# huangnengCSU/longcallR

Measured on AMD Instinct MI355X. Metric: candidate_sites_per_sec, higher is better.
Workload: dtype u8 in, u32 counts, f64 likelihoods, i64 fixed-point phase scores

## Files before the change

### longcallr_amd/csrc/k4_enum.hip

```cpp
#include <climits>
#include <type_traits>
#include "k4_dev.h"
#include "k4_kernels.h"

#ifndef ENUM_OCC
#define ENUM_OCC 3
#endif
namespace {

struct EnumTile { int32_t slot; uint32_t e0, ne; };
__device__ __forceinline__ EnumTile enum_tile_of(const PhaseDev& P, const EnumSpan* __restrict__ spans, int n_spans, uint32_t per, bool winner) {
  EnumTile t;
  const uint32_t bid = blockIdx.x;
  if (winner) { t.slot = spans[bid].slot; t.e0 = 0; t.ne = 1; return t; }
  const int lane = threadIdx.x & 63;
  int lo = 0, hi = n_spans;
  if (n_spans <= 4096) {
    const int step = (n_spans + 63) / 64;
    const int i1 = lane * step;
    const unsigned long long m1 = __ballot(i1 < n_spans && spans[min(i1, n_spans - 1)].tile0 <= bid);
    const int seg = __popcll(m1) - 1;
    lo = seg * step; hi = min(n_spans, lo + step);
    const int i2 = lo + lane;
    const unsigned long long m2 = __ballot(i2 < hi && spans[min(i2, n_spans - 1)].tile0 <= bid);
    lo = lo + __popcll(m2) - 1;
  } else {
    while (hi - lo > 1) { const int mid = (lo + hi) >> 1; if (spans[mid].tile0 <= bid) lo = mid; else hi = mid; }
  }
  t.slot = spans[lo].slot;
  const uint32_t n = 1u << P.reg[t.slot].S;
  t.e0 = (bid - spans[lo].tile0) * per;
  t.ne = min(per, n - t.e0);
  return t;
}

#ifdef ENUM_PROF
#define ENUM_PT(i) do { if (threadIdx.x == 0) atomicMax(&P.tie_ctr[i], (unsigned long long)((long long)wall_clock64() - prof_t0)); } while (0)
#else
#define ENUM_PT(i) do { } while (0)
#endif
__global__ void __launch_bounds__(64 * ENUM_WAVES)
k4_enum_resolve(PhaseDev P, const EnumSpan* __restrict__ spans, const int64_t* __restrict__ job_base, const long long* __restrict__ job_obj,
                const int64_t* __restrict__ st_base, const unsigned long long* __restrict__ st_words) {
  extern __shared__ __attribute__((aligned(16))) uint8_t lds[];
  const long long prof_t0 = (long long)wall_clock64(); (void)prof_t0;
  const int slot = spans[blockIdx.x].slot;
  const RegionDev rd = P.reg[slot];
  const int tid = threadIdx.x, nt = blockDim.x, lane = tid & 63, wave = tid >> 6;
  const int R = rd.R, S = rd.S;
  const uint32_t E = (uint32_t)P.prow_ptr[rd.rp_off + R];
  const uint32_t n_jobs = 1u << S;
// ... 359 lines not shown
  if (tid == 0) s_prof = 0;
  __syncthreads();
  if (tid == 0 && dif) s_prof = ((unsigned long long)(((long long)wall_clock64() - prof_t5) & 0xfffff) << 24) | ((unsigned long long)min(max(max(s_tloc[0], s_tloc[1]), max(s_tloc[2], s_tloc[3])) >> 4, 4095u) << 12) | min(max(max(s_tfull[0], s_tfull[1]), max(s_tfull[2], s_tfull[3])) >> 4, 4095u);
#endif
  const uint32_t we = s_win;
  const unsigned long long m0 = ld_st(we, nk);
  const uint32_t dneg = (uint32_t)m0, eta0 = (uint32_t)(m0 >> 32), etap = (uint32_t)ld_st(we, nk + 1);
  for (int i = tid; i < S; i += nt) {
    P.st_delta[rd.snp_off + i] = (int8_t)(((dneg >> i) & 1u) ? -1 : 1);
    P.st_eta[rd.snp_off + i] = (int8_t)(((eta0 >> i) & 1u) ? 0 : (((etap >> i) & 1u) ? 1 : -1));
  }
  for (int row = tid; row < R; row += nt) P.st_sigma[rd.sig_off + row] = (int8_t)(((ld_st(we, (uint32_t)row >> 6) >> (row & 63)) & 1ull) ? -1 : 1);
  if (tid == 0) P.st_obj[slot] = best;
#ifdef ENUM_PROF
  __syncthreads();
  if (tid == 0) atomicMax(&P.tie_ctr[7], ((unsigned long long)(((long long)wall_clock64() - prof_t0) & 0xfffff) << 44) | s_prof);
#endif
}

__device__ __forceinline__ int enum_incl_scan(int v) {
  v += __builtin_amdgcn_update_dpp(0, v, 0x111, 0xf, 0xf, false);
  v += __builtin_amdgcn_update_dpp(0, v, 0x112, 0xf, 0xf, false);
  v += __builtin_amdgcn_update_dpp(0, v, 0x114, 0xf, 0xf, false);
  v += __builtin_amdgcn_update_dpp(0, v, 0x118, 0xf, 0xf, false);
  v += __builtin_amdgcn_update_dpp(0, v, 0x142, 0xa, 0xf, false);
  v += __builtin_amdgcn_update_dpp(0, v, 0x143, 0xc, 0xf, false);
  return v;
}

__device__ __forceinline__ bool enum_tie_row_flips(const int row, const uint32_t sneg, const uint32_t dneg, const uint32_t eta0, const uint32_t etap,
                                                   const uint16_t* rp, const uint16_t* ent16, const double* lut) {
// ... 305 lines not shown
      job_obj[job_base[t.slot] + e] = total;
    }
    wave_lds_sync();
  };
  for (uint32_t kk = wave; kk < ne; kk += ENUM_WAVES) run_restart(t.e0 + kk);
  n_tie_f64 = (uint32_t)wave_sum_ll((long long)n_tie_f64); n_tie_flip = (uint32_t)wave_sum_ll((long long)n_tie_flip); n_tie_unres = (uint32_t)wave_sum_ll((long long)n_tie_unres);
  if (lane == 0) {
    if (n_tie_f64) TIE_COUNT(P.tie_ctr, TIE_SIGMA_F64, (unsigned long long)n_tie_f64);
    if (n_tie_flip) TIE_COUNT(P.tie_ctr, TIE_SIGMA_FLIPS, (unsigned long long)n_tie_flip);
    if (n_tie_unres) TIE_COUNT(P.tie_ctr, TIE_SIGMA_UNRES, (unsigned long long)n_tie_unres);
    if (n_dtie) TIE_COUNT(P.tie_ctr, TIE_DELTA_UNRES, (unsigned long long)n_dtie);
    if (n_step) TIE_COUNT(P.tie_ctr, TIE_STEP_UNRES, (unsigned long long)n_step);
  }
}

__device__ __forceinline__ uint32_t enum_spread8(uint32_t x) { x = (x | (x << 4)) & 0x0F0Fu; x = (x | (x << 2)) & 0x3333u; x = (x | (x << 1)) & 0x5555u; return x; }
__device__ __forceinline__ int enum_mad24(int a, int b, int c) { int d; asm("v_mad_i32_i24 %0, %1, %2, %3" : "=v"(d) : "v"(a), "v"(b), "v"(c)); return d; }

#ifndef ENUM_BITS_OCC
#define ENUM_BITS_OCC 2
#endif
__global__ void __launch_bounds__(64 * ENUM_WAVES, ENUM_BITS_OCC)
k4_enum_bits(PhaseDev P, const EnumSpan* __restrict__ spans, int32_t n_spans, uint32_t per, const int64_t* __restrict__ job_base,
             long long* __restrict__ job_obj, const int64_t* __restrict__ st_base, unsigned long long* __restrict__ st_words,
             long long* __restrict__ region_best, uint32_t* __restrict__ redo, uint32_t redo_cap) {
  extern __shared__ __attribute__((aligned(16))) uint8_t lds[];
  const EnumTile t = enum_tile_of(P, spans, n_spans, per, false);
  const RegionDev rd = P.reg[t.slot];
  const int R = rd.R, S = rd.S;
  const uint32_t E = (uint32_t)P.prow_ptr[rd.rp_off + R];
  const EnumLayout L = enum_layout(R, E, true, (uint32_t)S);
  const int Sp = (int)enum_bits_sp((uint32_t)S);
  uint2* wl2 = (uint2*)lds;
  double* lut = (double*)(lds + L.lut);
  uint2* csr = (uint2*)(lds + L.csr);
  uint32_t* csc = (uint32_t*)(lds + L.csc);
  uint16_t* rp = (uint16_t*)(lds + L.rp); uint16_t* first_row = (uint16_t*)(lds + L.first_row);
  uint16_t* ent16 = (uint16_t*)(lds + L.ent16);
  const int tid = threadIdx.x, nt = blockDim.x;
  const uint32_t c = enum_chunk(E);
  __shared__ long long s_cF[32], s_cW[32], s_cRef[32], s_cVar[32], s_het[32];
  __shared__ uint8_t s_live[32];
  if (tid < 32) {
    const long long w = tid < 31 ? P.lut.f1e[tid] - P.lut.fe[tid] : 0;
    wl2[tid] = make_uint2((uint32_t)w & 0x7fffffu, (uint32_t)(w >> 23) & 0xffffffu);
  }
  if (tid < 64) lut[tid] = (tid & 31) < 31 ? (tid < 32 ? P.lut64->le[tid] : P.lut64->l1e[tid - 32]) : 0.0;
  const int32_t* g_rp = P.prow_ptr + rd.rp_off;
  for (int r = tid; r <= R; r += nt) rp[r] = (uint16_t)g_rp[r];
  __shared__ int32_t cps[33];
  if (tid <= S && tid < 33) cps[tid] = P.ccol_ptr[rd.cp_off + tid];
  int eta_init = 0;
  if (tid < 32) {
    long long cF = 0, cW = 0, cRef = 0, cVar = 0, het = 0; bool live = false;
    if (tid < S) {
      const long long* sc = P.snp_const + 4ll * (rd.snp_off + tid);
      cF = sc[0]; cW = sc[1]; cRef = sc[2] + P.lut.f_homref; cVar = sc[3] + P.lut.f_homvar;
      const int n = P.ccol_ptr[rd.cp_off + tid + 1] - P.ccol_ptr[rd.cp_off + tid];
      het = P.lut.f_het0 - (long long)n * P.lut.f_log2;
      live = P.snp_fp[rd.snp_off + tid] != 0 && n > 0;
      eta_init = init_genotype(P.snp_vt[rd.snp_off + tid]);
    }
    s_cF[tid] = cF; s_cW[tid] = cW; s_cRef[tid] = cRef; s_cVar[tid] = cVar; s_het[tid] = het; s_live[tid] = live ? 1 : 0;
  }
  __shared__ uint32_t s_e0i, s_epi;
  if (tid < 64) {
    const uint32_t a = (uint32_t)__ballot(tid < S && tid < 32 && eta_init == 0), b = (uint32_t)__ballot(tid < S && tid < 32 && eta_init == 1);
    if (tid == 0) { s_e0i = a; s_epi = b; }
  }
  __syncthreads();
  for (int e = tid; e < (int)E; e += nt) {
    const uint32_t cv = P.cval[rd.e_off + e];
    int col = 0;
    for (int i = 0; i < S; i++) col += (int)((uint32_t)e >= (uint32_t)cps[i + 1]);
    csc[e] = (uint32_t)P.crow[rd.e_off + e] | ((uint32_t)col << 16) | ((cv & 32u) << 16) | ((cv & 31u) << 22) | 0x80000000u;
  }
  uint16_t* const perm = (uint16_t*)(lds + L.pos);
  uint16_t* const gof = perm + ((R + 3) & ~3);
  uint16_t* const kidx = (uint16_t*)(lds + L.state);
  __shared__ int s_cnt[3];
  __shared__ int s_lstart[32];
  __syncthreads();
  if (tid < 64) {
// ... 13 lines not shown
#pragma unroll
        for (int Lk = 2; Lk < 32; Lk++) {
          if (Lk <= S) {
            const unsigned long long bm = __ballot(n == Lk);
            if (n == Lk) kidx[r] = (uint16_t)(tot[Lk] + __popcll(bm & lt));
            tot[Lk] += __popcll(bm);
          }
        }
      }
    }
    int mine = 0;
#pragma unroll
    for (int Lk = 2; Lk < 32; Lk++) if (ln == Lk) mine = tot[Lk];
    int longer = 0;
    for (int Lk = 31; Lk >= 2; Lk--) { const int tl = __shfl(mine, Lk, 64); if (ln == Lk) s_lstart[ln] = longer; longer += tl; }
    if (ln == 0) { s_cnt[0] = longer; s_cnt[2] = nS; }
  }
  __syncthreads();
  const int nM = s_cnt[0], nS = s_cnt[2], nG = (nM + 63) >> 6;
  for (int r = tid; r < R; r += nt) {
    const int n = min(31, (int)rp[r + 1] - (int)rp[r]);
    if (n >= 2) perm[s_lstart[n] + kidx[r]] = (uint16_t)r;
  }
  __syncthreads();
  if (tid < 64) {
    int carry = 0;
    for (int g0 = 0; g0 <= nG; g0 += 64) {
      const int g = g0 + tid;
      const int len = g < nG ? min(31, (int)rp[perm[64 * g] + 1] - (int)rp[perm[64 * g]]) : 0;
      const int inc = wave_incl_scan(len);
      if (g <= nG) gof[g] = (uint16_t)(carry + inc - len);
// ... 9 lines not shown
    if (e0 == e1) continue;
    int at, step;
    if (e1 - e0 >= 2) {
      const int k = s_lstart[min(31, e1 - e0)] + kidx[r];
      at = 64 * (int)gof[k >> 6] + (k & 63); step = 64;
    } else { perm[nM + kidx[r]] = (uint16_t)r; at = eM + kidx[r]; step = 1; }
    for (int e = e0; e < e1; e++) {
      const uint32_t v = P.pval[rd.e_off + e];
      const uint32_t meta = (uint32_t)P.pcol[rd.e_off + e] | (v & 32u) | (e + 1 == e1 ? 64u : 0u) | 128u;
      const uint2 w = wl2[v & 31u];
      csr[at + (e - e0) * step] = make_uint2(w.x | (meta << 24), w.y);
      ent16[e] = (uint16_t)((meta & 63u) | ((v & 31u) << 6) | (e + 1 == e1 ? 0x800u : 0u));
    }
  }
  __syncthreads();
  const int lane = tid & 63, wave = tid >> 6;
  uint8_t* const wst = lds + L.state + wave * L.stride;
  uint8_t* const sg8 = wst;
  unsigned long long* const Macc = (unsigned long long*)(wst + ((R + 15) & ~7u));
  uint2* const mt = (uint2*)(Macc + 8 * Sp);
  uint32_t* const ms = (uint32_t*)(mt + 32);
  uint32_t* const tq = ms + 24;
  uint32_t* const tq_n = tq + ENUM_TQ;
  const int c0 = min((int)E, lane * (int)c), c1 = min((int)E, (lane + 1) * (int)c);
  const int n_del = (int)min(c, E);
  const uint32_t smask = S >= 32 ? 0xffffffffu : ((1u << S) - 1u);
  const uint32_t e0_init = s_e0i, ep_init = s_epi;
  const int nk = (R + 63) / 64;
  unsigned long long* const st_reg = st_words + st_base[t.slot];
  const uint32_t stw = enum_state_words((uint32_t)R);
  uint32_t n_tie_f64 = 0, n_tie_flip = 0, n_tie_unres = 0;
  uint32_t n_dtie = 0, n_step = 0;
  const int n_pass = (S + 7) >> 3;
  for (uint32_t g0 = 8u * wave; g0 < t.ne; g0 += 8u * ENUM_WAVES) {
    const uint32_t e_base = t.e0 + g0;
    const int nst = (int)min(8u, t.ne - g0);
    const uint32_t valid8 = (1u << nst) - 1u;
    if (lane < 8) { ms[lane] = (e_base + (uint32_t)lane) & smask; ms[8 + lane] = e0_init; ms[16 + lane] = ep_init; }
    {
      constexpr uint64_t G = 0x9E3779B97F4A7C15ULL;
      const uint64_t RG = (uint64_t)R * G;
      uint64_t a_row = rd.seed + ((uint64_t)S + (uint64_t)R + (uint64_t)e_base * (uint64_t)R + (uint64_t)lane + 1ull) * G;
// ... 179 lines not shown
              alo[s] += __umul24(b, wq[x].x); ahi[s] += __mul24((int)b, whi);
            }
          }
        }
        if (cur >= 0) flush();
      }
      wave_lds_sync();
      uint32_t any2 = 0, chg8 = 0;
      {
        const int s = lane >> 3;
        const uint32_t od = ms[s], oe0 = ms[8 + s], oep = ms[16 + s];
        uint32_t nd = od, ne0 = oe0, nep = oep;
        for (int p = 0; p < n_pass; p++) {
          const int i = 8 * p + (lane & 7);
          const bool in = i < S;
          const bool live = in && s_live[i & 31] != 0;
          int d_new = (int)((od >> i) & 1u), h_new = ((oe0 >> i) & 1u) ? 0 : (((oep >> i) & 1u) ? 1 : -1);
          bool changed = false, dtie = false;
          if (live && ((act >> s) & 1u)) {
            const long long M = (long long)Macc[s * Sp + i];
            const long long cF = s_cF[i], cW = s_cW[i], cRef = s_cRef[i], cVar = s_cVar[i], het = s_het[i];
            const long long N0 = cF + M + het, N1 = cF + cW - M + het;
            int ch = 0; long long nb = N0;
            if (N1 > nb) { ch = 1; nb = N1; }
            if (cRef > nb) { ch = 2; nb = cRef; }
            if (cVar > nb) { ch = 3; nb = cVar; }
            dtie = (int)(N0 == nb) + (int)(N1 == nb) + (int)(cRef == nb) + (int)(cVar == nb) > 1;
            const long long ncur = h_new == 0 ? N0 : (h_new == 1 ? cRef : cVar);
            changed = nb > ncur;
            if (ch == 1) d_new ^= 1;
            h_new = ch <= 1 ? 0 : (ch == 2 ? 1 : -1);
            objl[p] = ch <= 1 ? nb - het : (ch == 2 ? cRef - P.lut.f_homref : cVar - P.lut.f_homvar);
          }
          if (in) Macc[s * Sp + i] = 0;
          const unsigned long long bd = __ballot(in && d_new), b0 = __ballot(in && h_new == 0), bp = __ballot(in && h_new == 1);
          const unsigned long long bc = __ballot(changed), bt = __ballot(dtie);
// ... 95 lines not shown
        }
        if (lane == 0) { stp[nk] = (unsigned long long)ms[s] | ((unsigned long long)ms[8 + s] << 32); stp[nk + 1] = (unsigned long long)ms[16 + s]; stp[nk + 2] = sig; }
      }
      if (lane == 0) job_obj[job_base[t.slot] + e] = total;
    }
    wave_lds_sync();
  }
  n_tie_f64 = (uint32_t)wave_sum_ll((long long)n_tie_f64); n_tie_flip = (uint32_t)wave_sum_ll((long long)n_tie_flip); n_tie_unres = (uint32_t)wave_sum_ll((long long)n_tie_unres);
  if (lane == 0) {
    if (n_tie_f64) TIE_COUNT(P.tie_ctr, TIE_SIGMA_F64, (unsigned long long)n_tie_f64);
    if (n_tie_flip) TIE_COUNT(P.tie_ctr, TIE_SIGMA_FLIPS, (unsigned long long)n_tie_flip);
    if (n_tie_unres) TIE_COUNT(P.tie_ctr, TIE_SIGMA_UNRES, (unsigned long long)n_tie_unres);
    if (n_dtie) TIE_COUNT(P.tie_ctr, TIE_DELTA_UNRES, (unsigned long long)n_dtie);
    if (n_step) TIE_COUNT(P.tie_ctr, TIE_STEP_UNRES, (unsigned long long)n_step);
  }
}

__device__ __forceinline__ void enum_big_restart(const PhaseDev& P, const RegionDev& rd, int slot, uint32_t e, bool winner, int8_t* base, double* qrow,
                                                 long long* red, const long long* wl, unsigned long long* s_sig, const int64_t* __restrict__ job_base,
                                                 long long* __restrict__ job_obj, const int64_t* __restrict__ st_base, unsigned long long* __restrict__ st_words,
                                                 const MatView& mv, unsigned long long* macc = nullptr) {
  int8_t* sg = base; int8_t* dl = base + rd.R; int8_t* et = dl + rd.S;
  const int8_t* vt = P.snp_vt + rd.snp_off;
  const int lane = threadIdx.x & 63, wave = threadIdx.x >> 6;
  const uint32_t nk = (uint32_t)(rd.R + 63) / 64, sw = enum_state_words((uint32_t)rd.R);
  const bool keep = !winner && st_words && st_base[slot] >= 0;
  for (int i = threadIdx.x; i < rd.S; i += blockDim.x) { dl[i] = ((e >> i) & 1u) ? -1 : 1; et[i] = init_genotype(vt[i]); }
  const uint64_t ctr0 = (uint64_t)rd.S + (uint64_t)rd.R + (uint64_t)e * (uint64_t)rd.R;
  for (int row = threadIdx.x; row < rd.R; row += blockDim.x) sg[row] = u01(rd.seed, ctr0 + row) < 0.5 ? -1 : 1;
  __syncthreads();
// ... 173 lines not shown
        }
        __syncthreads();
        win = s_first;
      }
    }
  }
  if (tid == 0) win_e[slot] = win;
}
}

void launch_k4_enum_reg(unsigned n_blocks, size_t dyn_lds, hipStream_t s, const PhaseDev& P, const EnumSpan* spans, int32_t n_spans,
                        uint32_t per, const int64_t* job_base, long long* job_obj, const int64_t* st_base, unsigned long long* st_words,
                        long long* region_best, uint32_t* redo, uint32_t redo_cap) {
  hipLaunchKernelGGL(k4_enum_reg, dim3(n_blocks), dim3(64 * ENUM_WAVES), dyn_lds, s, P, spans, n_spans, per, job_base, job_obj, st_base, st_words, region_best, redo, redo_cap);
}
void launch_k4_enum_bits(unsigned n_blocks, size_t dyn_lds, hipStream_t s, const PhaseDev& P, const EnumSpan* spans, int32_t n_spans,
                         uint32_t per, const int64_t* job_base, long long* job_obj, const int64_t* st_base, unsigned long long* st_words,
                         long long* region_best, uint32_t* redo, uint32_t redo_cap) {
  hipLaunchKernelGGL(k4_enum_bits, dim3(n_blocks), dim3(64 * ENUM_WAVES), dyn_lds, s, P, spans, n_spans, per, job_base, job_obj, st_base, st_words, region_best, redo, redo_cap);
}
hipError_t k4_set_dyn_lds_once(const void* fn, int bytes, int slot);
void launch_k4_enum_redo(unsigned n_blocks, hipStream_t s, const PhaseDev& P, const uint32_t* redo, uint32_t redo_cap, int8_t* scratch, int32_t scratch_stride,
                         double* qrow, int64_t qrow_stride, const int64_t* job_base, long long* job_obj, const int64_t* st_base, unsigned long long* st_words,
                         uint32_t lds_bytes) {
  lds_bytes = std::min<uint32_t>(lds_bytes, 128 * 1024);
  if (lds_bytes > 32 * 1024 && k4_set_dyn_lds_once(reinterpret_cast<const void*>(&k4_enum_redo), 128 * 1024, 6) != hipSuccess) { (void)hipGetLastError(); lds_bytes = 32 * 1024; }
  hipLaunchKernelGGL(k4_enum_redo, dim3(n_blocks), dim3(LCR_BLOCK), lds_bytes, s, P, redo, redo_cap, scratch, scratch_stride, qrow, qrow_stride, job_base, job_obj, st_base, st_words, lds_bytes);
}
void launch_k4_enum_resolve(unsigned n_regions, size_t dyn_lds, hipStream_t s, const PhaseDev& P, const EnumSpan* spans, const int64_t* job_base,
                            const long long* job_obj, const int64_t* st_base, const unsigned long long* st_words) {
  hipLaunchKernelGGL(k4_enum_resolve, dim3(n_regions), dim3(64 * ENUM_WAVES), dyn_lds, s, P, spans, job_base, job_obj, st_base, st_words);
}
void launch_k4_enum_big(unsigned n_blocks, hipStream_t s, const PhaseDev& P, const EnumSpan* spans, int32_t n_spans, uint32_t per,
                        const int64_t* job_base, long long* job_obj, const uint32_t* win_e, const int64_t* st_base, unsigned long long* st_words,
// ... 8 lines not shown
```

### longcallr_amd/csrc/k4_kernels.h

```cpp
#pragma once
#include "k4_types.h"

struct EnumSpan { int32_t slot; uint32_t tile0; };
constexpr int ENUM_WAVES = 4;
constexpr uint32_t ENUM_LDS_MAX = 63 * 1024;

constexpr uint32_t ENUM_TQ = 126;
constexpr uint32_t ENUM_TCAP = 256;
#ifndef ENUM_BITS_PER_V
#define ENUM_BITS_PER_V 64
#endif
constexpr uint32_t ENUM_BITS_PER = ENUM_BITS_PER_V;
__host__ __device__ inline uint32_t enum_bits_sp(uint32_t S) { return (S + 7) & ~7u; }
__host__ __device__ inline uint32_t enum_bits_stride(uint32_t R, uint32_t S) { return ((R + 15) & ~7u) + 8 * 8 * enum_bits_sp(S) + 8 * 32 + 4 * 24 + 4 * (ENUM_TQ + 2); }
struct EnumLayout { uint32_t lut, csr, csc, rp, first_row, ent16, pos, state, stride, total; };
__host__ __device__ inline EnumLayout enum_layout(uint32_t R, uint32_t E, bool bits = false, uint32_t S = 32) {
  EnumLayout L;
  uint32_t o = 256;
  L.lut = o; o += 512;
  L.csr = o; o += 8 * (E + (bits ? 64 * (S < 31 ? S : 31) : 0));
  L.csc = o; o += 4 * E;
  L.rp = o; o += 2 * (R + 1);
  L.first_row = o; o += 2 * 65 + (bits ? 2 * 64 : 0);
  o = (o + 7) & ~7u;
  L.ent16 = o; o += 2 * ((E + 3) & ~3u);
  L.pos = o; if (bits) o += 2 * ((R + 3) & ~3u) + 2 * ((R + 4) & ~3u);
  o = (o + 15) & ~15u;
  L.state = o;
  L.stride = bits ? enum_bits_stride(R, S) : 8 * ((R + 63) / 64 + 1) + 8 * 32 + 4 * (ENUM_TQ + 2);
  o += ENUM_WAVES * L.stride;
  L.total = o;
  return L;
}
__host__ __device__ inline uint32_t enum_state_words(uint32_t R) { return (R + 63) / 64 + 3; }
__host__ __device__ inline uint32_t resolve_tlcap(uint32_t S) { return S >= 12 ? 4096u : (S < 6 ? 64u : (1u << S)); }
struct ResolveLayout { uint32_t lut, rp, ent16, pse, sg_ref, hetw, repmask, rowsnps, res, total; };
__host__ __device__ inline ResolveLayout resolve_layout(uint32_t R, uint32_t E, uint32_t S) {
  ResolveLayout L;
  const uint32_t nk = (R + 63) / 64;
  uint32_t o = 0;
  L.lut = o; o += 512;
  L.rp = o; o += 2 * (R + 2);
  o = (o + 15) & ~15u;
  L.ent16 = o; o += 2 * ((E + 7) & ~7u);
  o = (o + 15) & ~15u;
  L.pse = o; o += 8 * ((E + 8) & ~7u);
  L.sg_ref = o; o += 8 * (nk + 1);
  L.hetw = o; o += 8 * (nk + 1);
  L.repmask = o; o += 8 * nk * (S ? S : 1);
  L.rowsnps = o; o += 4 * (R + 1);
  o = (o + 7) & ~7u;
  L.res = o; o += ENUM_TCAP * 16 + 96 * 10 + 16 + 2 * resolve_tlcap(S);
  L.total = (o + 15) & ~15u;
  return L;
}
__host__ __device__ inline uint32_t enum_chunk(uint32_t E) { return E ? (E + 63) / 64 : 1; }

void launch_k4_enum_reg(unsigned n_blocks, size_t dyn_lds, hipStream_t s, const PhaseDev& P, const EnumSpan* spans, int32_t n_spans,
                        uint32_t per, const int64_t* job_base, long long* job_obj, const int64_t* st_base, unsigned long long* st_words,
                        long long* region_best, uint32_t* redo , uint32_t redo_cap);
void launch_k4_enum_bits(unsigned n_blocks, size_t dyn_lds, hipStream_t s, const PhaseDev& P, const EnumSpan* spans, int32_t n_spans,
                         uint32_t per, const int64_t* job_base, long long* job_obj, const int64_t* st_base, unsigned long long* st_words,
                         long long* region_best, uint32_t* redo, uint32_t redo_cap);
void launch_k4_enum_redo(unsigned n_blocks, hipStream_t s, const PhaseDev& P, const uint32_t* redo, uint32_t redo_cap, int8_t* scratch ,
                         int32_t scratch_stride, double* qrow , int64_t qrow_stride, const int64_t* job_base, long long* job_obj,
                         const int64_t* st_base, unsigned long long* st_words, uint32_t lds_bytes );
void launch_k4_enum_resolve(unsigned n_regions, size_t dyn_lds, hipStream_t s, const PhaseDev& P, const EnumSpan* spans, const int64_t* job_base,
                            const long long* job_obj, const int64_t* st_base, const unsigned long long* st_words);
void launch_k4_enum_big(unsigned n_blocks, hipStream_t s, const PhaseDev& P, const EnumSpan* spans, int32_t n_spans, uint32_t per,
                        const int64_t* job_base, long long* job_obj, const uint32_t* win_e ,
                        const int64_t* st_base , unsigned long long* st_words,
                        double* qrow , int64_t qrow_stride);
void launch_k4_enum_resolve_big(int32_t n, hipStream_t s, const PhaseDev& P, const EnumSpan* spans, const int64_t* job_base, const long long* job_obj,
                                const int64_t* st_base, const unsigned long long* st_words, uint32_t* win_e, double* terms ,
                                int64_t terms_stride);

constexpr int STAGE_THREADS = 256;
constexpr int STG_E = 8192, STG_R = 4096, STG_S = 512;
// ... 26 lines not shown
```

### longcallr_amd/csrc/k4_phase.hip

```cpp
#include <algorithm>
#include <chrono>
#include <cstdio>
#include <cstdlib>
#include <cmath>
#include <cstring>
#include <climits>
#include <map>
#include <thread>
#include <mutex>
#include <fcntl.h>
#include <sys/file.h>
#include <unistd.h>
#include <sys/stat.h>
#include <cerrno>

#include "k4_dev.h"
#include "k4_grid.h"
#include "k4_post.h"
#include "k4_kernels.h"

namespace {


struct HostLut {
// ... 565 lines not shown
    for (size_t k = 0; k < enum_slots.size(); k++) enum_slots[k] = (int32_t)(uint32_t)key[k];
  }
  HT("en:sorted");
  int32_t max_state = 0;
  for (int g : enum_slots) max_state = std::max(max_state, stat[g].R + 2 * in.snps(g));
  const int32_t stride = (max_state + 63) & ~63;
  P.scratch_stride = stride;
  const bool force_big = dbg.enum_force_big != 0;
  const bool force_stream = dbg.enum_force_stream != 0;
  enum { CL_STREAM, CL_BITS, CL_BIG, NCLS };
  std::vector<EnumSpan> spans[NCLS];
  spans[CL_STREAM].reserve(enum_slots.size()); spans[CL_BITS].reserve(enum_slots.size());
  size_t n_t[NCLS] = {0, 0, 0};
  const uint32_t per_of[NCLS] = {ENUM_STREAM_PER_WAVE * ENUM_WAVES, ENUM_BITS_PER, 1u};
  std::vector<int64_t>& job_base = enum_job_base; std::vector<int64_t>& st_base = enum_st_base;
  job_base.assign(ng, 0); st_base.assign(ng, 0);
  int64_t nj = 0, st_words = 0, big_words = 0, big_emax = 0;
  uint32_t lds_need[NCLS] = {0, 0, 0}, res_lds[NCLS] = {0, 0, 0};
  std::vector<int32_t> post_slots, post_slots_b, post_slots_c;
  post_slots.reserve(enum_slots.size());
  for (int g : enum_slots) {
    const int S = in.snps(g);
    const StageStat& st = stat[g];
    const EnumLayout EL_stream = enum_layout(st.R, st.E), EL_bits = enum_layout(st.R, st.E, true, (uint32_t)std::min(S, 32));
    const bool use_bits = !force_stream && S <= 31 && EL_bits.total <= ENUM_LDS_MAX;
    const EnumLayout EL = use_bits ? EL_bits : EL_stream;
    const uint32_t RL = resolve_layout((uint32_t)st.R, (uint32_t)st.E, (uint32_t)S).total;
    int cls = CL_BIG;
    if (!force_big && st.R < 65536 && st.E < 65536 && S <= 31 && EL.total <= ENUM_LDS_MAX && RL <= ENUM_LDS_MAX && st.max_rows <= 64)
      cls = use_bits ? CL_BITS : CL_STREAM;
    if (cls != CL_BIG && (int64_t)((uint64_t)1 << std::min(S, 62)) * enum_state_words((uint32_t)st.R) > ((int64_t)1 << 27)) cls = CL_BIG;
    if (cls != CL_BIG) { lds_need[cls] = std::max(lds_need[cls], EL.total); res_lds[cls] = std::max(res_lds[cls], RL); }
    job_base[g] = nj;
    const uint64_t n = 1ull << S;
    st_base[g] = -1;
    if (cls != CL_BIG) { st_base[g] = st_words; st_words += (int64_t)n * enum_state_words((uint32_t)st.R); }
    else if ((int64_t)n * enum_state_words((uint32_t)st.R) <= ((int64_t)1 << 26) - big_words) {
      st_base[g] = st_words; st_words += (int64_t)n * enum_state_words((uint32_t)st.R); big_words += (int64_t)n * enum_state_words((uint32_t)st.R);
      big_emax = std::max<int64_t>(big_emax, st.E);
    }
    if (n_t[cls] + (n + per_of[cls] - 1) / per_of[cls] > 0x7fffffffull) { if (c.err) *c.err = "too many enumeration restarts for one launch"; return LCR_E_ARG; }
    spans[cls].push_back({g, (uint32_t)n_t[cls]});
    n_t[cls] += (size_t)((n + per_of[cls] - 1) / per_of[cls]);
    nj += (int64_t)n;
    if (!c.host_post[g] && !c.grid_post[g]) (cls == CL_BITS ? post_slots_b : (cls == CL_BIG ? post_slots_c : post_slots)).push_back(g);
    if (c.prof && cls == CL_BIG) fprintf(stderr, "[phase]   global-memory enumeration region %d: R %d E %d S %d max_rows %d max_n %d, LDS image %u B\n", g, st.R, st.E, S, st.max_rows, st.max_n, EL.total);
  }
  if (c.prof) fprintf(stderr, "[phase]   enumeration classes: bit states %zu regions / %zu tiles, streaming %zu / %zu, global %zu / %zu\n",
                      spans[CL_BITS].size(), n_t[CL_BITS], spans[CL_STREAM].size(), n_t[CL_STREAM], spans[CL_BIG].size(), n_t[CL_BIG]);
  size_t n_w[NCLS], s_off[NCLS], n_spans = 0;
  for (int k = 0; k < NCLS; k++) { n_w[k] = spans[k].size(); s_off[k] = n_spans; n_spans += n_w[k]; }
  const size_t ns = enum_slots.size(), nps_a = post_slots.size(), nps_b = post_slots_b.size(), nps_c = post_slots_c.size(), nps = nps_a + nps_b + nps_c;
  const size_t off_jb_al = (n_spans * sizeof(EnumSpan) + 7) & ~(size_t)7;
  const size_t off_sb = off_jb_al + (size_t)ng * 8;
  const size_t up_bytes = off_sb + (size_t)ng * 8 + (ns + nps) * 4;
  HT("en:classes");
  PCHK(d_en_st.reserve((size_t)std::max<int64_t>(st_words, 1) * 8));
  PCHK(d_en_job.reserve(up_bytes + 64));
  PCHK(d_en_obj.reserve((size_t)nj * 8 + (size_t)ng * 8 + (size_t)ng * 8 + 64));
  PCHK(h_en_up.reserve(up_bytes + 64));
  uint8_t* const up = h_en_up.as<uint8_t>();
  for (int k = 0; k < NCLS; k++) memcpy(up + s_off[k] * sizeof(EnumSpan), spans[k].data(), n_w[k] * sizeof(EnumSpan));
  memcpy(up + off_jb_al, job_base.data(), (size_t)ng * 8);
  memcpy(up + off_sb, st_base.data(), (size_t)ng * 8);
  memcpy(up + off_sb + (size_t)ng * 8, enum_slots.data(), ns * 4);
  memcpy(up + off_sb + (size_t)ng * 8 + ns * 4, post_slots.data(), nps_a * 4);
  memcpy(up + off_sb + (size_t)ng * 8 + (ns + nps_a) * 4, post_slots_b.data(), nps_b * 4);
  memcpy(up + off_sb + (size_t)ng * 8 + (ns + nps_a + nps_b) * 4, post_slots_c.data(), nps_c * 4);
  PCHK(hipMemcpyAsync(d_en_job.p, up, up_bytes, hipMemcpyHostToDevice, stream));
  HT("en:up_q");
  const EnumSpan* d_sp = d_en_job.as<EnumSpan>();
  const int64_t* d_jb = (const int64_t*)(d_en_job.as<uint8_t>() + off_jb_al);
  const int64_t* d_sb = (const int64_t*)(d_en_job.as<uint8_t>() + off_sb);
  const int32_t* d_sl = (const int32_t*)(d_en_job.as<uint8_t>() + off_sb + (size_t)ng * 8);
  const int32_t* d_psl = d_sl + ns;
  long long* d_obj = d_en_obj.as<long long>();
  uint32_t* d_win = (uint32_t*)(d_obj + nj);
  const size_t n_big_blocks = std::max(n_t[CL_BIG], n_w[CL_BIG]);
  const bool full_ties = dbg.tie_arith >= 3;
  int32_t max_rows_any = 1;
  for (int g : enum_slots) max_rows_any = std::max(max_rows_any, stat[g].R);
  const int64_t qstride = ((int64_t)2 * max_rows_any + 15) & ~(int64_t)15;
  const size_t n_scr_blocks = n_big_blocks + 2 * (size_t)REDO_GRID;
  PCHK(d_en_scr.reserve((size_t)stride * n_scr_blocks + 64));
  P.scratch = d_en_scr.as<int8_t>();
  if (full_ties) PCHK(d_en_qrow.reserve((size_t)qstride * n_scr_blocks * 8 + 64));
  uint32_t* const redo_a = full_ties ? d_en_redo.as<uint32_t>() : nullptr;
  uint32_t* const redo_b = full_ties ? d_en_redo.as<uint32_t>() + 4 + 2 * REDO_CAP : nullptr;
  double* const qrow_all = full_ties ? d_en_qrow.as<double>() : nullptr;
// ... 7 lines not shown
  long long* const d_rbest = d_en_rbest.as<long long>();
  unsigned long long* const d_st = d_en_st.as<unsigned long long>();
  const uint32_t post_lds = c.post_lds; const PostIn& pin = c.pin; const PostLut& plut = c.plut;
  auto launch = [&](const size_t* cnt, const uint32_t* win) -> hipError_t {
    const bool fork = cnt[CL_STREAM] && (cnt[CL_BITS] || cnt[CL_BIG]);
    hipStream_t const qb = fork ? aux : stream;
    hipError_t e = hipSuccess;
    if (fork) { if ((e = hipEventRecord(ev_fork, stream)) != hipSuccess) return e; if ((e = hipStreamWaitEvent(aux, ev_fork, 0)) != hipSuccess) return e; }
    if (cnt[CL_STREAM]) {
      launch_k4_enum_reg((unsigned)cnt[CL_STREAM], lds_need[CL_STREAM], stream, P, d_sp + s_off[CL_STREAM], (int32_t)n_w[CL_STREAM], per_of[CL_STREAM], d_jb, d_obj, d_sb, d_st, d_rbest, redo_a, REDO_CAP);
      if (!win) {
        launch_redo(redo_a, 0, stream);
        launch_k4_enum_resolve((unsigned)n_w[CL_STREAM], res_lds[CL_STREAM], stream, P, d_sp + s_off[CL_STREAM], d_jb, d_obj, d_sb, d_st);
      }
    }
    if (cnt[CL_BITS]) launch_k4_enum_bits((unsigned)cnt[CL_BITS], lds_need[CL_BITS], qb, P, d_sp + s_off[CL_BITS], (int32_t)n_w[CL_BITS], per_of[CL_BITS], d_jb, d_obj, d_sb, d_st, d_rbest, redo_b, REDO_CAP);
    if (!win && c.async_mode) {
      if (cnt[CL_STREAM]) { if ((e = hipEventRecord(ev_gate[0], stream)) != hipSuccess) return e; gate_set[0] = true; }
      if (fork && cnt[CL_BITS]) { if ((e = hipEventRecord(ev_gate[1], qb)) != hipSuccess) return e; gate_set[1] = true; }
      else if (!fork && cnt[CL_BITS]) { if ((e = hipEventRecord(ev_gate[0], stream)) != hipSuccess) return e; gate_set[0] = true; }
    }
    if (!win) {
      if (nps_a && (e = launch_k4_post(2 * LCR_BLOCK, (unsigned)nps_a, post_lds, stream, pin, d_psl, (int32_t)nps_a, plut)) != hipSuccess) return e;
      if (cnt[CL_BITS]) { launch_redo(redo_b, 1, qb); launch_k4_enum_resolve((unsigned)n_w[CL_BITS], res_lds[CL_BITS], qb, P, d_sp + s_off[CL_BITS], d_jb, d_obj, d_sb, d_st); }
      if (nps_b && (e = launch_k4_post(2 * LCR_BLOCK, (unsigned)nps_b, post_lds, qb, pin, d_psl + nps_a, (int32_t)nps_b, plut)) != hipSuccess) return e;
    }
    if (cnt[CL_BIG]) launch_k4_enum_big((unsigned)cnt[CL_BIG], qb, P, d_sp + s_off[CL_BIG], (int32_t)n_w[CL_BIG], per_of[CL_BIG], d_jb, d_obj, win, d_sb, d_st, qrow_all, qstride);
    if (fork) { if ((e = hipEventRecord(ev_join, aux)) != hipSuccess) return e; if ((e = hipStreamWaitEvent(stream, ev_join, 0)) != hipSuccess) return e; }
    return e;
  };
  PCHK(launch(n_t, nullptr));
// ... 346 lines not shown
```

### longcallr_amd/csrc/lcr_phase_host.h

```cpp
#pragma once
#include <string>
#include <atomic>
#include <functional>
#include <memory>
#include <semaphore.h>
#include <thread>

#include "lcr_dev.h"
#include "k4_types.h"

struct PhaseInputs {
  int32_t n_regions = 0, n_rows = 0;
  int64_t nnz = 0;
  const int32_t* row_region_off = nullptr;
  const int32_t* cand_region_off = nullptr;
  const int64_t* region_start0 = nullptr;
  const int64_t* region_e_off = nullptr;
  const int64_t* d_row_ptr = nullptr;
  const int32_t* d_col = nullptr;
  const uint8_t* d_val = nullptr;
  const uint32_t* d_row_links = nullptr;
  std::vector<lcr_candidate>* cand = nullptr;
  const lcr_candidate* d_cand = nullptr;
  const int32_t* d_cand_off = nullptr;
// ... 75 lines not shown
  std::string lock_dir;
  std::vector<int8_t> haplotag;
  std::vector<uint8_t> assignment;
  std::vector<uint32_t> phase_set;
  std::vector<double> objective;
  const int8_t* r_haplotag = nullptr;
  const uint8_t* r_assignment = nullptr;
  const uint32_t* r_phase_set = nullptr;
  DevBuf d_reg, d_prow_ptr, d_pcol, d_pval, d_ccol_ptr, d_crow, d_cval, d_snp, d_snp_const, d_cur, d_prow_src;
  DevBuf d_grid_ctl, d_grid_tot;
  DevBuf d_st_enum, d_st_chain, d_read_rec, d_lut64, d_tie, d_prof_clk;
  bool lut64_ready = false;
  DevBuf d_ch_desc, d_ch_slots, d_ch_tbl, d_ch_adj, d_ch_part, d_ch_snpi, d_ch_snpb, d_ch_q, d_ch_info, d_ch_rowi, d_ch_enti, d_ch_work, d_ch_macc, d_ch_sig;
  DevBuf d_spec_sig, d_spec_de, d_spec_res, d_pk, d_bt;
  DevBuf d_tie_flag, d_tie_q, d_tie_ch, d_tie_terms;
  DevBuf d_en_job, d_en_obj, d_en_st, d_en_rbest, d_en_scr, d_en_qrow, d_en_redo, d_en_terms;
  DevBuf d_gp_snp, d_gp_ent, d_gp_part;
  HostBuf h_stat, h_res, h_cand_obj, h_census, h_en_up, h_ch_up;
  HostBuf h_row_ptr, h_col, h_val, h_links, h_st_enum, h_st_chain;
  unsigned long long tie_census[TIE_NCTR] = {0, 0, 0, 0, 0, 0, 0, 0};
  bool read_rec_stale = false;
  hipStream_t side = nullptr;
  hipEvent_t ev_in = nullptr, ev_csr = nullptr, ev_fork = nullptr, ev_join = nullptr;
  hipStream_t aux = nullptr;
  hipStream_t main_q = nullptr, q_first = nullptr;
  hipEvent_t ev_gate[2] = {nullptr, nullptr};
  bool gate_set[2] = {false, false};
  hipError_t gate_stream(hipStream_t s) {
    if (!pending) return hipSuccess;
    for (int k = 0; k < 2; k++) if (gate_set[k]) { hipError_t e = hipStreamWaitEvent(s, ev_gate[k], 0); if (e != hipSuccess) return e; }
    return hipSuccess;
  }
  hipEvent_t ev_user = nullptr;
  bool pending = false;
  struct Pending {
    int ng = 0; bool any_host_post = false;
    std::vector<int32_t> cand_off; std::vector<uint8_t> host_post;
    size_t res_ps = 0, res_tag = 0, res_asg = 0, hc_obj = 0;
    std::vector<lcr_candidate>* cand = nullptr;
  } pend;
  int settle(std::string* err);
  HostPool* pool = nullptr;
  void* work = nullptr;
  ChainDev chain_dev{};
  std::vector<ChainDesc> chain_desc;
  std::vector<uint64_t> enum_keys;
  std::vector<int64_t> enum_job_base, enum_st_base;
  int ld_blocks(const PhaseInputs& in, int region, std::vector<int32_t>* off, std::vector<int32_t>* snps, hipStream_t s, std::string* err);
  void free_work();
  int run(const PhaseInputs& in, const lcr_params& p, hipStream_t s, std::string* err);
  int open_queues(PhaseCall& c), size_buffers(PhaseCall& c), stage(PhaseCall& c), classify(PhaseCall& c), wait_sizes(PhaseCall& c);
  int launch_enum(PhaseCall& c), launch_chain(PhaseCall& c), launch_gpost(PhaseCall& c), report_prof(PhaseCall& c), host_epilogue(PhaseCall& c);
  bool mark_pending(PhaseCall& c);
  void release() {
    for (hipStream_t* q : {&side, &aux, &main_q}) { if (*q) (void)hipStreamDestroy(*q); *q = nullptr; }
    for (hipEvent_t* e : {&ev_in, &ev_csr, &ev_fork, &ev_join, &ev_user, &ev_gate[0], &ev_gate[1]}) { if (*e) (void)hipEventDestroy(*e); *e = nullptr; }
    gate_set[0] = gate_set[1] = false;
    pending = false;
    delete pool; pool = nullptr;
    free_work();
  }
};
// ... 1 lines not shown
```

Measured before the change: 5.953 billion.

## Build per-region LDS image once and copy it into enum_bits tiles

Splits the per-region LDS setup (LUT, CSR/CSC, row permutation, per-SNP constants) out of k4_enum_bits into a new k4_enum_image kernel that runs once per region and writes the finished LDS state to a global image buffer. Each enum_bits tile then bulk-loads that image with unrolled 16-byte loads instead of recomputing the setup. The tiles-per-block count is halved so more blocks share each image. This removes redundant setup work but adds an extra launch, global memory traffic and a serial dependency between the two kernels.

Result: faster. 6.034 billion (median of 6 runs) (+1.4%).

```diff
diff --git a/longcallr_amd/csrc/k4_enum.hip b/longcallr_amd/csrc/k4_enum.hip
--- a/longcallr_amd/csrc/k4_enum.hip
+++ b/longcallr_amd/csrc/k4_enum.hip
@@ -34,7 +34,7 @@
   return t;
 }
 
-#ifdef ENUM_PROF
+#if defined(ENUM_PROF) && ENUM_PROF != 2
 #define ENUM_PT(i) do { if (threadIdx.x == 0) atomicMax(&P.tie_ctr[i], (unsigned long long)((long long)wall_clock64() - prof_t0)); } while (0)
 #else
 #define ENUM_PT(i) do { } while (0)
@@ -424,7 +424,7 @@
   if (tid == 0) P.st_obj[slot] = best;
 #ifdef ENUM_PROF
   __syncthreads();
-  if (tid == 0) atomicMax(&P.tie_ctr[7], ((unsigned long long)(((long long)wall_clock64() - prof_t0) & 0xfffff) << 44) | s_prof);
+  if (tid == 0 && ENUM_PROF != 2) atomicMax(&P.tie_ctr[7], ((unsigned long long)(((long long)wall_clock64() - prof_t0) & 0xfffff) << 44) | s_prof);
 #endif
 }
 
@@ -760,33 +760,22 @@
   }
 }
 
-__device__ __forceinline__ uint32_t enum_spread8(uint32_t x) { x = (x | (x << 4)) & 0x0F0Fu; x = (x | (x << 2)) & 0x3333u; x = (x | (x << 1)) & 0x5555u; return x; }
-__device__ __forceinline__ int enum_mad24(int a, int b, int c) { int d; asm("v_mad_i32_i24 %0, %1, %2, %3" : "=v"(d) : "v"(a), "v"(b), "v"(c)); return d; }
-
-#ifndef ENUM_BITS_OCC
-#define ENUM_BITS_OCC 2
-#endif
-__global__ void __launch_bounds__(64 * ENUM_WAVES, ENUM_BITS_OCC)
-k4_enum_bits(PhaseDev P, const EnumSpan* __restrict__ spans, int32_t n_spans, uint32_t per, const int64_t* __restrict__ job_base,
-             long long* __restrict__ job_obj, const int64_t* __restrict__ st_base, unsigned long long* __restrict__ st_words,
-             long long* __restrict__ region_best, uint32_t* __restrict__ redo, uint32_t redo_cap) {
+__global__ void __launch_bounds__(ENUM_IMAGE_THREADS)
+k4_enum_image(PhaseDev P, const EnumSpan* __restrict__ spans, const int64_t* __restrict__ img_base, uint8_t* __restrict__ img) {
   extern __shared__ __attribute__((aligned(16))) uint8_t lds[];
-  const EnumTile t = enum_tile_of(P, spans, n_spans, per, false);
-  const RegionDev rd = P.reg[t.slot];
+  const int32_t slot = spans[blockIdx.x].slot;
+  const RegionDev rd = P.reg[slot];
   const int R = rd.R, S = rd.S;
   const uint32_t E = (uint32_t)P.prow_ptr[rd.rp_off + R];
   const EnumLayout L = enum_layout(R, E, true, (uint32_t)S);
-  const int Sp = (int)enum_bits_sp((uint32_t)S);
   uint2* wl2 = (uint2*)lds;
   double* lut = (double*)(lds + L.lut);
   uint2* csr = (uint2*)(lds + L.csr);
   uint32_t* csc = (uint32_t*)(lds + L.csc);
-  uint16_t* rp = (uint16_t*)(lds + L.rp); uint16_t* first_row = (uint16_t*)(lds + L.first_row);
+  uint16_t* rp = (uint16_t*)(lds + L.rp);
   uint16_t* ent16 = (uint16_t*)(lds + L.ent16);
   const int tid = threadIdx.x, nt = blockDim.x;
-  const uint32_t c = enum_chunk(E);
-  __shared__ long long s_cF[32], s_cW[32], s_cRef[32], s_cVar[32], s_het[32];
-  __shared__ uint8_t s_live[32];
+  __shared__ __attribute__((aligned(16))) EnumBitsCst s_c;
   if (tid < 32) {
     const long long w = tid < 31 ? P.lut.f1e[tid] - P.lut.fe[tid] : 0;
     wl2[tid] = make_uint2((uint32_t)w & 0x7fffffu, (uint32_t)(w >> 23) & 0xffffffu);
@@ -807,12 +796,11 @@
       live = P.snp_fp[rd.snp_off + tid] != 0 && n > 0;
       eta_init = init_genotype(P.snp_vt[rd.snp_off + tid]);
     }
-    s_cF[tid] = cF; s_cW[tid] = cW; s_cRef[tid] = cRef; s_cVar[tid] = cVar; s_het[tid] = het; s_live[tid] = live ? 1 : 0;
-  }
-  __shared__ uint32_t s_e0i, s_epi;
+    s_c.cF[tid] = cF; s_c.cW[tid] = cW; s_c.cRef[tid] = cRef; s_c.cVar[tid] = cVar; s_c.het[tid] = het; s_c.live[tid] = live ? 1 : 0;
+  }
   if (tid < 64) {
     const uint32_t a = (uint32_t)__ballot(tid < S && tid < 32 && eta_init == 0), b = (uint32_t)__ballot(tid < S && tid < 32 && eta_init == 1);
-    if (tid == 0) { s_e0i = a; s_epi = b; }
+    if (tid == 0) { s_c.e0i = a; s_c.epi = b; }
   }
   __syncthreads();
   for (int e = tid; e < (int)E; e += nt) {
@@ -856,7 +844,7 @@
     for (int Lk = 2; Lk < 32; Lk++) if (ln == Lk) mine = tot[Lk];
     int longer = 0;
     for (int Lk = 31; Lk >= 2; Lk--) { const int tl = __shfl(mine, Lk, 64); if (ln == Lk) s_lstart[ln] = longer; longer += tl; }
-    if (ln == 0) { s_cnt[0] = longer; s_cnt[2] = nS; }
+    if (ln == 0) { s_cnt[0] = longer; s_cnt[2] = nS; s_c.nM = (uint32_t)longer; s_c.nS = (uint32_t)nS; }
   }
   __syncthreads();
   const int nM = s_cnt[0], nS = s_cnt[2], nG = (nM + 63) >> 6;
@@ -896,6 +884,68 @@
     }
   }
   __syncthreads();
+  uint4* const dst = (uint4*)(img + img_base[slot]);
+  const uint32_t n16 = L.state / 16;
+  for (uint32_t i = tid; i < n16; i += nt) dst[i] = ((const uint4*)lds)[i];
+  for (uint32_t i = tid; i < (uint32_t)(sizeof(EnumBitsCst) / 16); i += nt) dst[n16 + i] = ((const uint4*)&s_c)[i];
+}
+
+#if defined(ENUM_PROF) && ENUM_PROF == 2
+#define ENUM_BITS_SPLIT() do { __syncthreads(); if (threadIdx.x == 0) { const unsigned long long te = (unsigned long long)wall_clock64(); \
+    atomicAdd(&P.tie_ctr[0], prof_ts - prof_t0); atomicAdd(&P.tie_ctr[1], te - prof_ts); atomicMax(&P.tie_ctr[2], ~prof_t0); atomicMax(&P.tie_ctr[3], te); \
+    atomicMax(&P.tie_ctr[4], te - prof_t0); atomicAdd(&P.tie_ctr[5], 1ull); atomicAdd(&P.tie_ctr[6], te); atomicMax(&P.tie_ctr[7], prof_ts - prof_t0); } } while (0)
+#else
+#define ENUM_BITS_SPLIT() do { } while (0)
+#endif
+__device__ __forceinline__ uint32_t enum_spread8(uint32_t x) { x = (x | (x << 4)) & 0x0F0Fu; x = (x | (x << 2)) & 0x3333u; x = (x | (x << 1)) & 0x5555u; return x; }
+__device__ __forceinline__ int enum_mad24(int a, int b, int c) { int d; asm("v_mad_i32_i24 %0, %1, %2, %3" : "=v"(d) : "v"(a), "v"(b), "v"(c)); return d; }
+
+#ifndef ENUM_BITS_OCC
+#define ENUM_BITS_OCC 2
+#endif
+__global__ void __launch_bounds__(64 * ENUM_WAVES, ENUM_BITS_OCC)
+k4_enum_bits(PhaseDev P, const EnumSpan* __restrict__ spans, int32_t n_spans, uint32_t per, const int64_t* __restrict__ job_base,
+             long long* __restrict__ job_obj, const int64_t* __restrict__ st_base, unsigned long long* __restrict__ st_words,
+             long long* __restrict__ region_best, uint32_t* __restrict__ redo, uint32_t redo_cap, const int64_t* __restrict__ img_base,
+             const uint8_t* __restrict__ img) {
+  extern __shared__ __attribute__((aligned(16))) uint8_t lds[];
+  const unsigned long long prof_t0 = (unsigned long long)wall_clock64(); (void)prof_t0;
+  const EnumTile t = enum_tile_of(P, spans, n_spans, per, false);
+  const RegionDev rd = P.reg[t.slot];
+  const int R = rd.R, S = rd.S;
+  const uint32_t E = (uint32_t)P.prow_ptr[rd.rp_off + R];
+  const EnumLayout L = enum_layout(R, E, true, (uint32_t)S);
+  const int Sp = (int)enum_bits_sp((uint32_t)S);
+  uint2* wl2 = (uint2*)lds;
+  double* lut = (double*)(lds + L.lut);
+  uint2* csr = (uint2*)(lds + L.csr);
+  uint32_t* csc = (uint32_t*)(lds + L.csc);
+  uint16_t* rp = (uint16_t*)(lds + L.rp);
+  uint16_t* ent16 = (uint16_t*)(lds + L.ent16);
+  const int tid = threadIdx.x, nt = blockDim.x;
+  const uint32_t c = enum_chunk(E);
+  __shared__ __attribute__((aligned(16))) EnumBitsCst s_c;
+  {
+    const uint4* const src = (const uint4*)(img + img_base[t.slot]);
+    const uint32_t n16 = L.state / 16, n_all = n16 + (uint32_t)(sizeof(EnumBitsCst) / 16);
+    for (uint32_t i0 = 0; i0 < n_all; i0 += 8u * (uint32_t)nt) {
+      uint4 v[8];
+#pragma unroll
+      for (int u = 0; u < 8; u++) { const uint32_t i = i0 + (uint32_t)(u * nt + tid); v[u] = i < n_all ? src[i] : make_uint4(0, 0, 0, 0); }
+#pragma unroll
+      for (int u = 0; u < 8; u++) {
+        const uint32_t i = i0 + (uint32_t)(u * nt + tid);
+        if (i < n16) ((uint4*)lds)[i] = v[u];
+        else if (i < n_all) ((uint4*)&s_c)[i - n16] = v[u];
+      }
+    }
+  }
+  uint16_t* const perm = (uint16_t*)(lds + L.pos);
+  uint16_t* const gof = perm + ((R + 3) & ~3);
+  __syncthreads();
+  const unsigned long long prof_ts = (unsigned long long)wall_clock64(); (void)prof_ts;
+  const int nM = (int)s_c.nM, nS = (int)s_c.nS, nG = (nM + 63) >> 6;
+  const int eM = 64 * (int)gof[nG];
   const int lane = tid & 63, wave = tid >> 6;
   uint8_t* const wst = lds + L.state + wave * L.stride;
   uint8_t* const sg8 = wst;
@@ -907,7 +957,7 @@
   const int c0 = min((int)E, lane * (int)c), c1 = min((int)E, (lane + 1) * (int)c);
   const int n_del = (int)min(c, E);
   const uint32_t smask = S >= 32 ? 0xffffffffu : ((1u << S) - 1u);
-  const uint32_t e0_init = s_e0i, ep_init = s_epi;
+  const uint32_t e0_init = s_c.e0i, ep_init = s_c.epi;
   const int nk = (R + 63) / 64;
   unsigned long long* const st_reg = st_words + st_base[t.slot];
   const uint32_t stw = enum_state_words((uint32_t)R);
@@ -1117,12 +1167,12 @@
         for (int p = 0; p < n_pass; p++) {
           const int i = 8 * p + (lane & 7);
           const bool in = i < S;
-          const bool live = in && s_live[i & 31] != 0;
+          const bool live = in && s_c.live[i & 31] != 0;
           int d_new = (int)((od >> i) & 1u), h_new = ((oe0 >> i) & 1u) ? 0 : (((oep >> i) & 1u) ? 1 : -1);
           bool changed = false, dtie = false;
           if (live && ((act >> s) & 1u)) {
             const long long M = (long long)Macc[s * Sp + i];
-            const long long cF = s_cF[i], cW = s_cW[i], cRef = s_cRef[i], cVar = s_cVar[i], het = s_het[i];
+            const long long cF = s_c.cF[i], cW = s_c.cW[i], cRef = s_c.cRef[i], cVar = s_c.cVar[i], het = s_c.het[i];
             const long long N0 = cF + M + het, N1 = cF + cW - M + het;
             int ch = 0; long long nb = N0;
             if (N1 > nb) { ch = 1; nb = N1; }
@@ -1248,6 +1298,7 @@
     if (n_dtie) TIE_COUNT(P.tie_ctr, TIE_DELTA_UNRES, (unsigned long long)n_dtie);
     if (n_step) TIE_COUNT(P.tie_ctr, TIE_STEP_UNRES, (unsigned long long)n_step);
   }
+  ENUM_BITS_SPLIT();
 }
 
 __device__ __forceinline__ void enum_big_restart(const PhaseDev& P, const RegionDev& rd, int slot, uint32_t e, bool winner, int8_t* base, double* qrow,
@@ -1451,10 +1502,15 @@
                         long long* region_best, uint32_t* redo, uint32_t redo_cap) {
   hipLaunchKernelGGL(k4_enum_reg, dim3(n_blocks), dim3(64 * ENUM_WAVES), dyn_lds, s, P, spans, n_spans, per, job_base, job_obj, st_base, st_words, region_best, redo, redo_cap);
 }
+void launch_k4_enum_image(unsigned n_regions, size_t dyn_lds, hipStream_t s, const PhaseDev& P, const EnumSpan* spans, const int64_t* img_base,
+                          uint8_t* img) {
+  hipLaunchKernelGGL(k4_enum_image, dim3(n_regions), dim3(ENUM_IMAGE_THREADS), dyn_lds, s, P, spans, img_base, img);
+}
 void launch_k4_enum_bits(unsigned n_blocks, size_t dyn_lds, hipStream_t s, const PhaseDev& P, const EnumSpan* spans, int32_t n_spans,
                          uint32_t per, const int64_t* job_base, long long* job_obj, const int64_t* st_base, unsigned long long* st_words,
-                         long long* region_best, uint32_t* redo, uint32_t redo_cap) {
-  hipLaunchKernelGGL(k4_enum_bits, dim3(n_blocks), dim3(64 * ENUM_WAVES), dyn_lds, s, P, spans, n_spans, per, job_base, job_obj, st_base, st_words, region_best, redo, redo_cap);
+                         long long* region_best, uint32_t* redo, uint32_t redo_cap, const int64_t* img_base, const uint8_t* img) {
+  hipLaunchKernelGGL(k4_enum_bits, dim3(n_blocks), dim3(64 * ENUM_WAVES), dyn_lds, s, P, spans, n_spans, per, job_base, job_obj, st_base, st_words, region_best, redo, redo_cap,
+                     img_base, img);
 }
 hipError_t k4_set_dyn_lds_once(const void* fn, int bytes, int slot);
 void launch_k4_enum_redo(unsigned n_blocks, hipStream_t s, const PhaseDev& P, const uint32_t* redo, uint32_t redo_cap, int8_t* scratch, int32_t scratch_stride,
diff --git a/longcallr_amd/csrc/k4_kernels.h b/longcallr_amd/csrc/k4_kernels.h
--- a/longcallr_amd/csrc/k4_kernels.h
+++ b/longcallr_amd/csrc/k4_kernels.h
@@ -8,7 +8,7 @@
 constexpr uint32_t ENUM_TQ = 126;
 constexpr uint32_t ENUM_TCAP = 256;
 #ifndef ENUM_BITS_PER_V
-#define ENUM_BITS_PER_V 64
+#define ENUM_BITS_PER_V 32
 #endif
 constexpr uint32_t ENUM_BITS_PER = ENUM_BITS_PER_V;
 __host__ __device__ inline uint32_t enum_bits_sp(uint32_t S) { return (S + 7) & ~7u; }
@@ -32,6 +32,15 @@
   L.total = o;
   return L;
 }
+struct EnumBitsCst {
+  long long cF[32], cW[32], cRef[32], cVar[32], het[32];
+  uint32_t e0i, epi;
+  uint32_t nM, nS;
+  uint8_t live[32];
+  uint32_t pad_[4];
+};
+static_assert(sizeof(EnumBitsCst) % 16 == 0, "the image is copied in 16-byte words");
+__host__ __device__ inline uint32_t enum_image_bytes(uint32_t R, uint32_t E, uint32_t S) { return enum_layout(R, E, true, S).state + (uint32_t)sizeof(EnumBitsCst); }
 __host__ __device__ inline uint32_t enum_state_words(uint32_t R) { return (R + 63) / 64 + 3; }
 __host__ __device__ inline uint32_t resolve_tlcap(uint32_t S) { return S >= 12 ? 4096u : (S < 6 ? 64u : (1u << S)); }
 struct ResolveLayout { uint32_t lut, rp, ent16, pse, sg_ref, hetw, repmask, rowsnps, res, total; };
@@ -59,9 +68,14 @@
 void launch_k4_enum_reg(unsigned n_blocks, size_t dyn_lds, hipStream_t s, const PhaseDev& P, const EnumSpan* spans, int32_t n_spans,
                         uint32_t per, const int64_t* job_base, long long* job_obj, const int64_t* st_base, unsigned long long* st_words,
                         long long* region_best, uint32_t* redo , uint32_t redo_cap);
+#ifndef ENUM_IMAGE_THREADS
+#define ENUM_IMAGE_THREADS 1024
+#endif
+void launch_k4_enum_image(unsigned n_regions, size_t dyn_lds, hipStream_t s, const PhaseDev& P, const EnumSpan* spans, const int64_t* img_base,
+                          uint8_t* img);
 void launch_k4_enum_bits(unsigned n_blocks, size_t dyn_lds, hipStream_t s, const PhaseDev& P, const EnumSpan* spans, int32_t n_spans,
                          uint32_t per, const int64_t* job_base, long long* job_obj, const int64_t* st_base, unsigned long long* st_words,
-                         long long* region_best, uint32_t* redo, uint32_t redo_cap);
+                         long long* region_best, uint32_t* redo, uint32_t redo_cap, const int64_t* img_base, const uint8_t* img);
 void launch_k4_enum_redo(unsigned n_blocks, hipStream_t s, const PhaseDev& P, const uint32_t* redo, uint32_t redo_cap, int8_t* scratch ,
                          int32_t scratch_stride, double* qrow , int64_t qrow_stride, const int64_t* job_base, long long* job_obj,
                          const int64_t* st_base, unsigned long long* st_words, uint32_t lds_bytes );
diff --git a/longcallr_amd/csrc/k4_phase.hip b/longcallr_amd/csrc/k4_phase.hip
--- a/longcallr_amd/csrc/k4_phase.hip
+++ b/longcallr_amd/csrc/k4_phase.hip
@@ -603,8 +603,9 @@
   size_t n_t[NCLS] = {0, 0, 0};
   const uint32_t per_of[NCLS] = {ENUM_STREAM_PER_WAVE * ENUM_WAVES, ENUM_BITS_PER, 1u};
   std::vector<int64_t>& job_base = enum_job_base; std::vector<int64_t>& st_base = enum_st_base;
-  job_base.assign(ng, 0); st_base.assign(ng, 0);
-  int64_t nj = 0, st_words = 0, big_words = 0, big_emax = 0;
+  std::vector<int64_t>& img_base = enum_img_base;
+  job_base.assign(ng, 0); st_base.assign(ng, 0); img_base.assign(ng, 0);
+  int64_t nj = 0, st_words = 0, big_words = 0, big_emax = 0, img_bytes = 0;
   uint32_t lds_need[NCLS] = {0, 0, 0}, res_lds[NCLS] = {0, 0, 0};
   std::vector<int32_t> post_slots, post_slots_b, post_slots_c;
   post_slots.reserve(enum_slots.size());
@@ -620,6 +621,7 @@
       cls = use_bits ? CL_BITS : CL_STREAM;
     if (cls != CL_BIG && (int64_t)((uint64_t)1 << std::min(S, 62)) * enum_state_words((uint32_t)st.R) > ((int64_t)1 << 27)) cls = CL_BIG;
     if (cls != CL_BIG) { lds_need[cls] = std::max(lds_need[cls], EL.total); res_lds[cls] = std::max(res_lds[cls], RL); }
+    if (cls == CL_BITS) { img_base[g] = img_bytes; img_bytes += enum_image_bytes((uint32_t)st.R, (uint32_t)st.E, (uint32_t)S); }
     job_base[g] = nj;
     const uint64_t n = 1ull << S;
     st_base[g] = -1;
@@ -642,9 +644,12 @@
   const size_t ns = enum_slots.size(), nps_a = post_slots.size(), nps_b = post_slots_b.size(), nps_c = post_slots_c.size(), nps = nps_a + nps_b + nps_c;
   const size_t off_jb_al = (n_spans * sizeof(EnumSpan) + 7) & ~(size_t)7;
   const size_t off_sb = off_jb_al + (size_t)ng * 8;
-  const size_t up_bytes = off_sb + (size_t)ng * 8 + (ns + nps) * 4;
+  const size_t off_ib = off_sb + (size_t)ng * 8;
+  const size_t off_sl = off_ib + (size_t)ng * 8;
+  const size_t up_bytes = off_sl + (ns + nps) * 4;
   HT("en:classes");
   PCHK(d_en_st.reserve((size_t)std::max<int64_t>(st_words, 1) * 8));
+  PCHK(d_en_img.reserve((size_t)std::max<int64_t>(img_bytes, 16)));
   PCHK(d_en_job.reserve(up_bytes + 64));
   PCHK(d_en_obj.reserve((size_t)nj * 8 + (size_t)ng * 8 + (size_t)ng * 8 + 64));
   PCHK(h_en_up.reserve(up_bytes + 64));
@@ -652,16 +657,18 @@
   for (int k = 0; k < NCLS; k++) memcpy(up + s_off[k] * sizeof(EnumSpan), spans[k].data(), n_w[k] * sizeof(EnumSpan));
   memcpy(up + off_jb_al, job_base.data(), (size_t)ng * 8);
   memcpy(up + off_sb, st_base.data(), (size_t)ng * 8);
-  memcpy(up + off_sb + (size_t)ng * 8, enum_slots.data(), ns * 4);
-  memcpy(up + off_sb + (size_t)ng * 8 + ns * 4, post_slots.data(), nps_a * 4);
-  memcpy(up + off_sb + (size_t)ng * 8 + (ns + nps_a) * 4, post_slots_b.data(), nps_b * 4);
-  memcpy(up + off_sb + (size_t)ng * 8 + (ns + nps_a + nps_b) * 4, post_slots_c.data(), nps_c * 4);
+  memcpy(up + off_ib, img_base.data(), (size_t)ng * 8);
+  memcpy(up + off_sl, enum_slots.data(), ns * 4);
+  memcpy(up + off_sl + ns * 4, post_slots.data(), nps_a * 4);
+  memcpy(up + off_sl + (ns + nps_a) * 4, post_slots_b.data(), nps_b * 4);
+  memcpy(up + off_sl + (ns + nps_a + nps_b) * 4, post_slots_c.data(), nps_c * 4);
   PCHK(hipMemcpyAsync(d_en_job.p, up, up_bytes, hipMemcpyHostToDevice, stream));
   HT("en:up_q");
   const EnumSpan* d_sp = d_en_job.as<EnumSpan>();
   const int64_t* d_jb = (const int64_t*)(d_en_job.as<uint8_t>() + off_jb_al);
   const int64_t* d_sb = (const int64_t*)(d_en_job.as<uint8_t>() + off_sb);
-  const int32_t* d_sl = (const int32_t*)(d_en_job.as<uint8_t>() + off_sb + (size_t)ng * 8);
+  const int64_t* d_ib = (const int64_t*)(d_en_job.as<uint8_t>() + off_ib);
+  const int32_t* d_sl = (const int32_t*)(d_en_job.as<uint8_t>() + off_sl);
   const int32_t* d_psl = d_sl + ns;
   long long* d_obj = d_en_obj.as<long long>();
   uint32_t* d_win = (uint32_t*)(d_obj + nj);
@@ -699,7 +706,11 @@
         launch_k4_enum_resolve((unsigned)n_w[CL_STREAM], res_lds[CL_STREAM], stream, P, d_sp + s_off[CL_STREAM], d_jb, d_obj, d_sb, d_st);
       }
     }
-    if (cnt[CL_BITS]) launch_k4_enum_bits((unsigned)cnt[CL_BITS], lds_need[CL_BITS], qb, P, d_sp + s_off[CL_BITS], (int32_t)n_w[CL_BITS], per_of[CL_BITS], d_jb, d_obj, d_sb, d_st, d_rbest, redo_b, REDO_CAP);
+    if (cnt[CL_BITS]) {
+      launch_k4_enum_image((unsigned)n_w[CL_BITS], lds_need[CL_BITS], qb, P, d_sp + s_off[CL_BITS], d_ib, d_en_img.as<uint8_t>());
+      launch_k4_enum_bits((unsigned)cnt[CL_BITS], lds_need[CL_BITS], qb, P, d_sp + s_off[CL_BITS], (int32_t)n_w[CL_BITS], per_of[CL_BITS], d_jb, d_obj, d_sb, d_st, d_rbest, redo_b, REDO_CAP,
+                          d_ib, d_en_img.as<uint8_t>());
+    }
     if (!win && c.async_mode) {
       if (cnt[CL_STREAM]) { if ((e = hipEventRecord(ev_gate[0], stream)) != hipSuccess) return e; gate_set[0] = true; }
       if (fork && cnt[CL_BITS]) { if ((e = hipEventRecord(ev_gate[1], qb)) != hipSuccess) return e; gate_set[1] = true; }
diff --git a/longcallr_amd/csrc/lcr_phase_host.h b/longcallr_amd/csrc/lcr_phase_host.h
--- a/longcallr_amd/csrc/lcr_phase_host.h
+++ b/longcallr_amd/csrc/lcr_phase_host.h
@@ -113,7 +113,7 @@
   DevBuf d_ch_desc, d_ch_slots, d_ch_tbl, d_ch_adj, d_ch_part, d_ch_snpi, d_ch_snpb, d_ch_q, d_ch_info, d_ch_rowi, d_ch_enti, d_ch_work, d_ch_macc, d_ch_sig;
   DevBuf d_spec_sig, d_spec_de, d_spec_res, d_pk, d_bt;
   DevBuf d_tie_flag, d_tie_q, d_tie_ch, d_tie_terms;
-  DevBuf d_en_job, d_en_obj, d_en_st, d_en_rbest, d_en_scr, d_en_qrow, d_en_redo, d_en_terms;
+  DevBuf d_en_job, d_en_obj, d_en_st, d_en_rbest, d_en_scr, d_en_qrow, d_en_redo, d_en_terms, d_en_img;
   DevBuf d_gp_snp, d_gp_ent, d_gp_part;
   HostBuf h_stat, h_res, h_cand_obj, h_census, h_en_up, h_ch_up;
   HostBuf h_row_ptr, h_col, h_val, h_links, h_st_enum, h_st_chain;
@@ -144,7 +144,7 @@
   ChainDev chain_dev{};
   std::vector<ChainDesc> chain_desc;
   std::vector<uint64_t> enum_keys;
-  std::vector<int64_t> enum_job_base, enum_st_base;
+  std::vector<int64_t> enum_job_base, enum_st_base, enum_img_base;
   int ld_blocks(const PhaseInputs& in, int region, std::vector<int32_t>* off, std::vector<int32_t>* snps, hipStream_t s, std::string* err);
   void free_work();
   int run(const PhaseInputs& in, const lcr_params& p, hipStream_t s, std::string* err);
```
